# JerryX1110/Robust-Video-Object-Segmentation

Measured on AMD Instinct MI355X. Metric: frames/sec, AOC-Net matching + calibration hot path (480p, 3 objects), higher is better.
Workload: dtype f32; 1 GPU; cfg2: 121x213 stride-4 maps (480p), O=4 (3 objects + background), K=16 proxies, C=100, 60-frame clips, MEM_EVERY=5 (pool R=1..12), 20 Lloyd iterations, local windows 2..12, 10 IA gates + 4 conditioning blocks; sequences_per_gpu=2, proxy_mode=reference

## Files before the change

robust-video-object-segmentation_amd/csrc/dense_split.hip:

```cpp
#include <atomic>
#include <type_traits>

#include "aoc_common.h"

namespace {

typedef _Float16 f16x8 __attribute__((ext_vector_type(8)));
typedef float f32x16 __attribute__((ext_vector_type(16)));

constexpr int SP_KS = 7;
constexpr int SP_K = SP_KS * 16;
constexpr int SP_HALF = SP_KS * 2;
constexpr int SP_REC = 2 * SP_HALF;
constexpr int SP_NORM_SLOT = 100;
constexpr int SP_REST_SLOT = 104;
constexpr float SP_SCALE = 1024.0f;
constexpr float SP_QCONST = 32768.0f;
constexpr float SP_UNSCALE = -1.0f / 524288.0f;
constexpr int SP_TILE = 32;
constexpr int SP_NB = 4;
constexpr int SP_NQ = 2;

static_assert(SP_NORM_SLOT + 4 <= SP_K && SP_NORM_SLOT / 16 == SP_KS - 1 && (SP_NORM_SLOT % 16) + 4 <= 8, "norm slots live in the low half of the last k-step");
static_assert(SP_REST_SLOT / 16 == SP_KS - 1 && SP_REST_SLOT % 16 == 8, "the rest-norm slots are the first two halves of the last k-step's high chunk");

template <bool TILED>
__global__ __launch_bounds__(256) void split_rows_kernel(const float *__restrict__ x, int64_t n, int C, uint4 *__restrict__ rec,
                                                          float *__restrict__ sqnorm, int32_t *__restrict__ overflow) {
    const int64_t idx = (int64_t)blockIdx.x * blockDim.x + threadIdx.x;
    int64_t row;
    int ks;
    if (TILED) {
        const int64_t tile = idx / (SP_KS * 32);
        const int rem = (int)(idx - tile * (SP_KS * 32));
        ks = rem >> 5;
        row = tile * 32 + (rem & 31);
        if (tile * 32 >= n) return;
    } else {
        row = idx / SP_KS;
        ks = (int)(idx - row * SP_KS);
        if (row >= n) return;
    }
    const bool live = row < n;
    const float *xr = x + (size_t)(live ? row : n - 1) * C;
    _Float16 hi[16], lo[16];
    bool bad = false;
    {
        const int c4k = C >> 2;
        float4 kv[4];
#pragma unroll
        for (int q = 0; q < 4; ++q) kv[q] = reinterpret_cast<const float4 *>(xr)[min(ks * 4 + q, c4k - 1)];
#pragma unroll
        for (int q = 0; q < 4; ++q) {
            const bool in = ks * 4 + q < c4k;
            const float e4[4] = {kv[q].x, kv[q].y, kv[q].z, kv[q].w};
#pragma unroll
            for (int u = 0; u < 4; ++u) {
                const float v = in ? e4[u] * SP_SCALE : 0.0f;
                bad |= !(fabsf(v) <= 65000.0f);
                hi[q * 4 + u] = (_Float16)v;
                lo[q * 4 + u] = (_Float16)(v - (float)hi[q * 4 + u]);
            }
        }
    }
    if (ks == SP_KS - 1) {
        float s = 0.0f, sl = 0.0f, hr3 = 0.0f, hr4 = 0.0f;
        float4 rv[SP_NORM_SLOT / 4];
        const int c4n = C >> 2;
#pragma unroll
        for (int t4 = 0; t4 < SP_NORM_SLOT / 4; ++t4) rv[t4] = reinterpret_cast<const float4 *>(xr)[t4 < c4n ? t4 : c4n - 1];
#pragma unroll
        for (int t4 = 0; t4 < SP_NORM_SLOT / 4; ++t4) {
            if (t4 < c4n) {
// ... 89 lines not shown
        if (obj < 0 && t < base + nt) { obj = o; local = (int)(nt - 1 - (t - base)); }
        base += nt;
    }
    if (e == 0) *n_tiles = (int32_t)base;
    int32_t id = -1;
    if (obj >= 0) {
        const int pos = local * SP_TILE + i;
        id = obj_rows[obj_offsets[obj] + (pos < counts[obj] ? pos : local * SP_TILE)];
    }
    tile_rows[e] = id;
    if (i == 0) tile_obj[t] = obj;
}

__device__ __forceinline__ float max16(const f32x16 &a) {
    float m0 = __builtin_fmaxf(__builtin_fmaxf(a[0], a[1]), a[2]);
    float m1 = __builtin_fmaxf(__builtin_fmaxf(a[3], a[4]), a[5]);
    float m2 = __builtin_fmaxf(__builtin_fmaxf(a[6], a[7]), a[8]);
    float m3 = __builtin_fmaxf(__builtin_fmaxf(a[9], a[10]), a[11]);
    float m4 = __builtin_fmaxf(__builtin_fmaxf(a[12], a[13]), a[14]);
    m0 = __builtin_fmaxf(__builtin_fmaxf(m0, m1), m2);
    m3 = __builtin_fmaxf(__builtin_fmaxf(m3, m4), a[15]);
    return __builtin_fmaxf(m0, m3);
}

__device__ __forceinline__ uint32_t ord_enc(float f) {
    const uint32_t u = __float_as_uint(f);
    return (u & 0x80000000u) ? ~u : (u | 0x80000000u);
}
__device__ __forceinline__ float ord_dec(uint32_t u) {
    if (u == 0u) return -INFINITY;
    return __uint_as_float((u & 0x80000000u) ? (u & 0x7fffffffu) : ~u);
}
__device__ __forceinline__ uint32_t load_relaxed(const uint32_t *p) {
    return __hip_atomic_load(p, __ATOMIC_RELAXED, __HIP_MEMORY_SCOPE_AGENT);
}

#ifdef AOC_DEV
__device__ unsigned long long aoc_dev_block_times[4096 * 6];
#endif
__device__ unsigned long long g_prune_stats[8];

__device__ __forceinline__ void glds16(const void *gsrc, uint32_t lds_dst) {
    unsigned keep;
    asm volatile("s_mov_b32 %0, m0\n\ts_mov_b32 m0, %2\n\ts_nop 0\n\tglobal_load_lds_dwordx4 %1, off\n\ts_mov_b32 m0, %0"
                 : "=&s"(keep) : "v"(gsrc), "s"(lds_dst) : "memory");
}
__device__ __forceinline__ void glds4(const void *gsrc, uint32_t lds_dst) {
    unsigned keep;
    asm volatile("s_mov_b32 %0, m0\n\ts_mov_b32 m0, %2\n\ts_nop 0\n\tglobal_load_lds_dword %1, off\n\ts_mov_b32 m0, %0"
                 : "=&s"(keep) : "v"(gsrc), "s"(lds_dst) : "memory");
}

constexpr int SP_NBUF = 2;
__host__ __device__ constexpr int sp_chunk_bytes(int nb) { return nb * SP_TILE * SP_REC * 16; }
__host__ __device__ constexpr int sp_ids_off(int nb) { return SP_NBUF * sp_chunk_bytes(nb); }
__host__ __device__ constexpr int sp_obj_off(int nb) { return sp_ids_off(nb) + 2 * 512; }
__host__ __device__ constexpr int sp_bnd_off(int nb) { return sp_obj_off(nb) + 4 * 256; }
__host__ __device__ constexpr int sp_lds_bytes(int nw, int nb) { return sp_bnd_off(nb) + nw * SP_NQ * 256; }
constexpr int SP_TILE_SLACK = 2;

template <int NW, int CKPT, int NB = SP_NB>
__global__ __launch_bounds__(NW * 64, NB == 2 ? 2 : 1) void dense_prune_kernel(const uint4 *__restrict__ qrec, const float *__restrict__ q2, int64_t m,
                                                                     const uint4 *__restrict__ prec, const int32_t *__restrict__ tile_rows,
                                                                     const int32_t *__restrict__ tile_obj, const int32_t *__restrict__ n_tiles_ptr,
                                                                     const int32_t *__restrict__ gate, const uint32_t *__restrict__ pmax_bits,
                                                                     int n_obj, uint32_t *__restrict__ gbest, int dbg_arg, int q_tiled) {
    if (*gate) return;
#ifdef AOC_DEV
    const int dbg = dbg_arg;
#else
    constexpr int dbg = 0;
    (void)dbg_arg;
#endif
    extern __shared__ __attribute__((aligned(16))) uint4 lds4[];
    static_assert(SP_NQ == 2 && ((NB == 4 && (NW == 8 || NW == 4)) || (NB == 2 && NW == 4)),
                  "the step structure below is written for 4 tiles x 2 query tiles x 8 (or 4) waves, or 2 tiles x 2 query tiles x 4 waves (two workgroups per CU)");
    constexpr int SP_CHUNK_BYTES = sp_chunk_bytes(NB), SP_IDS_OFF = sp_ids_off(NB), SP_OBJ_OFF = sp_obj_off(NB), SP_BND_OFF = sp_bnd_off(NB);
    static_assert(CKPT == 0 || CKPT == 3 || CKPT == 4, "checkpoint after 3 or 4 k-steps (rest norms in slots 104 / 105), or none");
    constexpr int SP_DMA_PER_WAVE = SP_CHUNK_BYTES / 1024 / NW;
    constexpr int W_ID0 = NW / 2, W_ID1 = NW - 1, W_OBJ = 1;
    const uint32_t lds_base = (uint32_t)reinterpret_cast<uintptr_t>(lds4);
    const char *lds_bytes = reinterpret_cast<const char *>(lds4);

    int bx, by;
    {
        const int nb = gridDim.x * gridDim.y, lin = blockIdx.y * gridDim.x + blockIdx.x;
        const int xcd = lin & 7, slot = lin >> 3, q = nb >> 3, r = nb & 7;
        const int v = (xcd < r ? xcd * (q + 1) : r * (q + 1) + (xcd - r) * q) + slot;
        by = v / gridDim.x;
        bx = v - by * gridDim.x;
    }
    const int n_tiles = *n_tiles_ptr;
    const int ns = gridDim.y;
    if (by >= n_tiles) return;
    const int n_mine = (n_tiles - by + ns - 1) / ns;
    const int n_chunks = (n_mine + NB - 1) / NB;

    const int lane = aoc_lane(), wave = __builtin_amdgcn_readfirstlane(threadIdx.x >> 6);
    const int col = lane & 31, h = lane >> 5;
    const int64_t wave_row0 = (int64_t)bx * (NW * SP_NQ * 32) + (int64_t)wave * (SP_NQ * 32);

    const float pmax = sqrtf(__uint_as_float(*pmax_bits)) * 1.001f;
    const float plmax = __uint_as_float(*(pmax_bits - 2));
    f16x8 bh[SP_NQ][SP_KS], bl[SP_NQ][SP_KS];
    float eps[SP_NQ];
    bool valid[SP_NQ];
#pragma unroll
    for (int iq = 0; iq < SP_NQ; ++iq) {
        const int64_t row = wave_row0 + iq * 32 + col;
        valid[iq] = row < m;
        const int64_t rr = valid[iq] ? row : 0;
        const uint4 *r = q_tiled ? qrec + (size_t)(rr >> 5) * (2 * SP_KS * 64) + h * 32 + (rr & 31) : qrec + (size_t)rr * SP_REC + h;
        const int ks_step = q_tiled ? 64 : 2, plane_step = q_tiled ? SP_KS * 64 : SP_HALF;
#pragma unroll
        for (int ks = 0; ks < SP_KS; ++ks) {
            uint4 u = r[ks * ks_step], v = r[plane_step + ks * ks_step];
            if (!valid[iq]) { u = make_uint4(0, 0, 0, 0); v = make_uint4(0, 0, 0, 0); }
            bh[iq][ks] = __builtin_bit_cast(f16x8, u);
            bl[iq][ks] = __builtin_bit_cast(f16x8, v);
        }
        const float ql_own = (float)bh[iq][SP_KS - 1][SP_NORM_SLOT % 16 + 3];
        if (h == 0) {
            bh[iq][SP_KS - 1][SP_NORM_SLOT % 16 + 3] = (_Float16)0.0f;
            bh[iq][SP_KS - 1][SP_NORM_SLOT % 16] = (_Float16)SP_QCONST;
            bh[iq][SP_KS - 1][SP_NORM_SLOT % 16 + 1] = (_Float16)SP_QCONST;
            bh[iq][SP_KS - 1][SP_NORM_SLOT % 16 + 2] = (_Float16)SP_QCONST;
        } else {
            if (CKPT != 3) bh[iq][SP_KS - 1][0] = (_Float16)0.0f;
            if (CKPT != 4) bh[iq][SP_KS - 1][1] = (_Float16)0.0f;
        }
        const float qn = valid[iq] ? sqrtf(q2[row]) : 0.0f;
        const float ql = valid[iq] ? __shfl(ql_own, col) : 0.0f;
        eps[iq] = (1026.0f * (qn * plmax + ql * pmax) + 8.0f * pmax * pmax + (CKPT != 0 ? 16.0f * qn * pmax : 0.0f) + 8.0f) * ((dbg & 64) ? 0.4f : 1.0f);
    }

    uint32_t dma_plan[SP_DMA_PER_WAVE];
#pragma unroll
    for (int k = 0; k < SP_DMA_PER_WAVE; ++k) {
        const int j = (wave * SP_DMA_PER_WAVE + k) * 64 + lane;
        const int r = j / SP_REC, pos = j - r * SP_REC;
        dma_plan[k] = ((uint32_t)r << 16) | (uint32_t)((pos ^ ((r >> 3) & 3)) * 16);
    }
    const char *prec_bytes = reinterpret_cast<const char *>(prec);
    auto dma_meta = [&](int chunk) {
        const int i0 = chunk * NB;
        if (wave == W_ID0 || (NB == 4 && wave == W_ID1)) {
            const int i = i0 + (wave == W_ID1 ? 2 : 0) + (lane >> 5);
            const int t = min(by + i * ns, n_tiles);
            glds4(tile_rows + (size_t)t * SP_TILE + (lane & 31), lds_base + SP_IDS_OFF + (chunk & 1) * 512 + (wave == W_ID1 ? 256 : 0));
        }
        if (wave == W_OBJ) glds4(tile_obj + min(by + (i0 + (lane & (NB - 1))) * ns, n_tiles), lds_base + SP_OBJ_OFF + (chunk & 3) * 256);
    };
    auto dma_rows = [&](int chunk) {
        const int32_t *ids = reinterpret_cast<const int32_t *>(lds_bytes + SP_IDS_OFF + (chunk & 1) * 512);
        const uint32_t dst = lds_base + (uint32_t)(chunk % SP_NBUF) * SP_CHUNK_BYTES + (uint32_t)(wave * SP_DMA_PER_WAVE) * 1024u;
        int id[SP_DMA_PER_WAVE];
#pragma unroll
        for (int k = 0; k < SP_DMA_PER_WAVE; ++k) id[k] = ids[dma_plan[k] >> 16];
#pragma unroll
        for (int k = 0; k < SP_DMA_PER_WAVE; ++k)
            glds16(prec_bytes + (size_t)(uint32_t)max(id[k], 0) * (SP_REC * 16) + (dma_plan[k] & 0xffffu), dst + (uint32_t)k * 1024u);
    };

    float best[SP_NQ], shared[SP_NQ];
    uint32_t grow[SP_NQ];
#pragma unroll
    for (int iq = 0; iq < SP_NQ; ++iq) {
        grow[iq] = valid[iq] ? (uint32_t)(wave_row0 + iq * 32 + col) * (uint32_t)n_obj : 0u;
        best[iq] = INFINITY;
        shared[iq] = INFINITY;
    }
    int cur = -1;
    unsigned n_rescored = 0, n_any = 0, n_seen = 0, n_dead = 0;
    unsigned long long cyc[6] = {0, 0, 0, 0, 0, 0};
    unsigned long long t_prev = 0;
    auto stamp = [&]() -> unsigned long long { return (dbg & 4096) ? __builtin_amdgcn_s_memtime() : 0ull; };
    auto dma_bound = [&]() {
#pragma unroll
        for (int iq = 0; iq < SP_NQ; ++iq) {
            unsigned keep;
            asm volatile("s_mov_b32 %0, m0\n\ts_mov_b32 m0, %2\n\ts_nop 0\n\tglobal_load_lds_dword %1, off sc1\n\ts_mov_b32 m0, %0"
                         : "=&s"(keep) : "v"(gbest + grow[iq] + max(cur, 0)), "s"(lds_base + SP_BND_OFF + (uint32_t)(wave * SP_NQ + iq) * 256u) : "memory");
        }
    };
    auto switch_object = [&](int o) {
        cur = o;
        uint32_t u[SP_NQ];
#pragma unroll
        for (int iq = 0; iq < SP_NQ; ++iq) u[iq] = load_relaxed(gbest + grow[iq] + cur);
#pragma unroll
        for (int iq = 0; iq < SP_NQ; ++iq) {
            best[iq] = valid[iq] ? -INFINITY : INFINITY;
            shared[iq] = valid[iq] ? ord_dec(u[iq]) : INFINITY;
        }
    };

#ifdef AOC_DEV
    const int blk_lin = blockIdx.y * gridDim.x + blockIdx.x;
    const bool blk_rec = (dbg & 32768) && threadIdx.x == 0 && blk_lin < 4096;
    if (blk_rec) aoc_dev_block_times[blk_lin * 6 + 0] = wall_clock64();
#endif
    dma_meta(0);
    dma_meta(1);
    __builtin_amdgcn_s_waitcnt(0x0f70);
    __builtin_amdgcn_s_barrier();
    dma_rows(0);
    __builtin_amdgcn_s_waitcnt(0x0f70);
    __builtin_amdgcn_s_barrier();

    const int xs = (col >> 3) & 3;
    const uint32_t row_off = (uint32_t)col * (SP_REC * 16);
    const uint32_t sw0 = row_off + (uint32_t)((h ^ xs) * 16), sw2 = row_off + (uint32_t)(((2 + h) ^ xs) * 16);
    auto frag = [&](const char *tile_base, int e) -> f16x8 {
        const uint32_t off = ((e & 2) ? sw2 : sw0) + (uint32_t)((e & ~3) * 16);
        return __builtin_bit_cast(f16x8, *reinterpret_cast<const uint4 *>(tile_base + off));
    };
    auto ks_of = [&](int kk) { return (kk + SP_KS - 1) % SP_KS; };
#ifdef AOC_DEV
    if (blk_rec) aoc_dev_block_times[blk_lin * 6 + 1] = wall_clock64();
#endif

    for (int s = 0; s < n_chunks; ++s) {
        const unsigned long long t_s0 = stamp();
        const int4 objs = *reinterpret_cast<const int4 *>(lds_bytes + SP_OBJ_OFF + (s & 3) * 256);
        const int bound_obj = (dbg & 32) ? -3 : cur;
        if (!(dbg & 32)) dma_bound();
        dma_meta(s + 2);
        if (!(dbg & 4)) dma_rows(s + 1);

        const char *chunk_base = lds_bytes + (s % SP_NBUF) * SP_CHUNK_BYTES;
        const int n_here = min(NB, n_mine - s * NB);
        f16x8 pre0 = frag(chunk_base, 2 * ks_of(0)), pre1 = frag(chunk_base, 2 * ks_of(1));
        const uint32_t objs_packed = (uint32_t)__builtin_amdgcn_readfirstlane((objs.x & 0xff) | ((objs.y & 0xff) << 8) | ((objs.z & 0xff) << 16) | ((objs.w & 0xff) << 24));
        t_prev = stamp();
        cyc[4] += t_prev - t_s0;
#pragma unroll 1
        for (int t = 0; t < n_here; ++t) {
            const char *tile_base = chunk_base + t * (SP_TILE * SP_REC * 16);
            const int o = (int)((objs_packed >> (8 * t)) & 0xffu);
            if (o != cur) switch_object(o);
            const unsigned long long t_0 = stamp();
            cyc[3] += t_0 - t_prev;
            f32x16 acc[SP_NQ];
#pragma unroll
            for (int iq = 0; iq < SP_NQ; ++iq)
#pragma unroll
                for (int r = 0; r < 16; ++r) acc[iq][r] = 0.0f;
            bool live[SP_NQ] = {true, true};
            if constexpr (CKPT == 0) {
                f16x8 af[3];
                af[0] = pre0;
                af[1] = pre1;
#pragma unroll
                for (int kk = 0; kk < SP_KS; ++kk) {
                    if (kk + 2 < SP_KS && !(dbg & 512)) af[(kk + 2) % 3] = frag(tile_base, 2 * ks_of(kk + 2));
#pragma unroll
                    for (int iq = 0; iq < SP_NQ; ++iq)
                        acc[iq] = __builtin_amdgcn_mfma_f32_32x32x16_f16(af[kk % 3], bh[iq][ks_of(kk)], acc[iq], 0, 0, 0);
                }
                if (t + 1 < n_here) {
                    pre0 = frag(tile_base + SP_TILE * SP_REC * 16, 2 * ks_of(0));
                    pre1 = frag(tile_base + SP_TILE * SP_REC * 16, 2 * ks_of(1));
                }
            } else {
                f16x8 af[3];
                af[0] = pre0;
                af[1] = frag(tile_base, 2 * ks_of(1));
                const uint32_t a6d0 = __builtin_bit_cast(uint4, pre0).x;
#pragma unroll
                for (int kk = 0; kk < CKPT; ++kk) {
                    if (kk + 2 < CKPT) af[(kk + 2) % 3] = frag(tile_base, 2 * ks_of(kk + 2));
#pragma unroll
                    for (int iq = 0; iq < SP_NQ; ++iq)
                        acc[iq] = __builtin_amdgcn_mfma_f32_32x32x16_f16(af[kk % 3], bh[iq][ks_of(kk)], acc[iq], 0, 0, 0);
                }
                if (t + 1 < n_here) pre0 = frag(tile_base + SP_TILE * SP_REC * 16, 2 * ks_of(0));
#pragma unroll
                for (int iq = 0; iq < SP_NQ; ++iq) {
                    const float cm = max16(acc[iq]);
                    live[iq] = (__builtin_amdgcn_ballot_w64(cm + eps[iq] >= __builtin_fmaxf(best[iq], shared[iq])) != 0ull) || (dbg & 128);
                    if (!live[iq]) n_dead += 1;
                }
                if (live[0] || live[1]) {
                    uint4 c4 = make_uint4(0u, 0u, 0u, 0u);
                    if (h == 1) c4.x = (CKPT == 3) ? ((a6d0 & 0x0000ffffu) ^ 0x00008000u) : ((a6d0 & 0xffff0000u) ^ 0x80000000u);
                    const f16x8 a6c = __builtin_bit_cast(f16x8, c4);
                    auto phase2 = [&](auto q0, auto q1) {
                        constexpr bool Q0 = decltype(q0)::value, Q1 = decltype(q1)::value;
                        f16x8 ar[3];
                        ar[0] = frag(tile_base, 2 * ks_of(CKPT));
                        ar[1] = frag(tile_base, 2 * ks_of(CKPT + 1));
                        if (Q0) acc[0] = __builtin_amdgcn_mfma_f32_32x32x16_f16(a6c, bh[0][SP_KS - 1], acc[0], 0, 0, 0);
                        if (Q1) acc[1] = __builtin_amdgcn_mfma_f32_32x32x16_f16(a6c, bh[1][SP_KS - 1], acc[1], 0, 0, 0);
#pragma unroll
                        for (int kk = CKPT; kk < SP_KS; ++kk) {
                            if (kk + 2 < SP_KS) ar[(kk + 2 - CKPT) % 3] = frag(tile_base, 2 * ks_of(kk + 2));
                            if (Q0) acc[0] = __builtin_amdgcn_mfma_f32_32x32x16_f16(ar[(kk - CKPT) % 3], bh[0][ks_of(kk)], acc[0], 0, 0, 0);
                            if (Q1) acc[1] = __builtin_amdgcn_mfma_f32_32x32x16_f16(ar[(kk - CKPT) % 3], bh[1][ks_of(kk)], acc[1], 0, 0, 0);
                        }
                    };
                    if (live[0] && live[1]) phase2(std::true_type{}, std::true_type{});
                    else if (live[0]) phase2(std::true_type{}, std::false_type{});
                    else phase2(std::false_type{}, std::true_type{});
                }
            }
            const unsigned long long t_1 = stamp();
            cyc[0] += t_1 - t_0;
            bool want[SP_NQ];
#pragma unroll
            for (int iq = 0; iq < SP_NQ; ++iq) {
                want[iq] = false;
                if (live[iq] && !(dbg & 256)) {
                    const float cm = max16(acc[iq]);
                    want[iq] = __builtin_amdgcn_ballot_w64(cm + eps[iq] >= __builtin_fmaxf(best[iq], shared[iq])) != 0ull;
                }
            }
            n_seen += 1;
            const unsigned long long t_2 = stamp();
            cyc[1] += t_2 - t_1;
            t_prev = t_2;
            if ((want[0] || want[1]) && !(dbg & 2)) {
                n_any += 1;
#pragma unroll
                for (int iq = 0; iq < SP_NQ; ++iq) {
                    if (want[iq]) {
                        n_rescored += 1;
                        if (dbg & 65536) {
                            if (cur == 0) cyc[0] += 1;
                            else if (cur == 1) cyc[1] += 1;
                            else if (cur == 2) cyc[2] += 1;
                        }
                        f16x8 ah[3], al[3];
#pragma unroll
                        for (int kk = 0; kk < 2; ++kk) {
                            ah[kk] = frag(tile_base, 2 * ks_of(kk));
                            al[kk] = frag(tile_base, 2 * SP_KS + 2 * ks_of(kk));
                        }
#pragma unroll
                        for (int kk = 0; kk < SP_KS; ++kk) {
                            if (kk + 2 < SP_KS) {
                                ah[(kk + 2) % 3] = frag(tile_base, 2 * ks_of(kk + 2));
                                al[(kk + 2) % 3] = frag(tile_base, 2 * SP_KS + 2 * ks_of(kk + 2));
                            }
                            acc[iq] = __builtin_amdgcn_mfma_f32_32x32x16_f16(ah[kk % 3], bl[iq][ks_of(kk)], acc[iq], 0, 0, 0);
                            acc[iq] = __builtin_amdgcn_mfma_f32_32x32x16_f16(al[kk % 3], bh[iq][ks_of(kk)], acc[iq], 0, 0, 0);
                        }
                        const float ex = max16(acc[iq]);
                        if (ex > best[iq]) {
                            best[iq] = ex;
                            if (ex > shared[iq] && !(dbg & 1)) atomicMax(gbest + grow[iq] + cur, ord_enc(ex));
                        }
                    }
                }
                t_prev = stamp();
                cyc[2] += t_prev - t_2;
            }
        }
        const unsigned long long t_s1 = stamp();

        __builtin_amdgcn_s_waitcnt(0x0f70);
        uint32_t seen[SP_NQ];
#pragma unroll
        for (int iq = 0; iq < SP_NQ; ++iq)
            seen[iq] = *reinterpret_cast<const volatile uint32_t *>(lds_bytes + SP_BND_OFF + (wave * SP_NQ + iq) * 256 + lane * 4);
        __builtin_amdgcn_s_waitcnt(0xc07f);
        if (!(dbg & 8)) __builtin_amdgcn_s_barrier();
        if (bound_obj == cur && cur >= 0) {
#pragma unroll
            for (int iq = 0; iq < SP_NQ; ++iq)
                if (valid[iq]) shared[iq] = __builtin_fmaxf(shared[iq], ord_dec(seen[iq]));
        }
        cyc[5] += stamp() - t_s1;
#ifdef AOC_DEV
        if (blk_rec && s == 0) aoc_dev_block_times[blk_lin * 6 + 2] = wall_clock64();
#endif
    }
#ifdef AOC_DEV
    if (blk_rec) {
        aoc_dev_block_times[blk_lin * 6 + 3] = wall_clock64();
        aoc_dev_block_times[blk_lin * 6 + 4] = n_seen;
        aoc_dev_block_times[blk_lin * 6 + 5] = n_rescored;
    }
#endif
    if (lane == 0) {
        atomicAdd(&g_prune_stats[0], (unsigned long long)n_seen * SP_NQ);
        atomicAdd(&g_prune_stats[1], (unsigned long long)n_rescored);
        atomicAdd(&g_prune_stats[2], (unsigned long long)n_any);
        atomicAdd(&g_prune_stats[3], (unsigned long long)n_seen);
        atomicAdd(&g_prune_stats[4], (unsigned long long)n_dead);
        if (dbg & (4096 | 65536)) {
            const int b = (dbg & 8192) ? 3 : 0;
            atomicAdd(&g_prune_stats[5], cyc[b]);
            atomicAdd(&g_prune_stats[6], cyc[b + 1]);
            atomicAdd(&g_prune_stats[7], cyc[b + 2]);
        }
    }
}

#ifndef AOC_DENSE_Q4
#define AOC_DENSE_Q4 0
#endif
#if defined(AOC_DEV) || AOC_DENSE_Q4
constexpr int Q4_NW = 4, Q4_NQ = 4;
#ifndef AOC_Q4_DBG
#define AOC_Q4_DBG 0
#endif
// ... 290 lines not shown

__global__ __launch_bounds__(256) void dense_split_finalize_kernel(uint32_t *__restrict__ gbest, int64_t m, int n_obj,
                                                                    const int32_t *__restrict__ counts, const int32_t *__restrict__ gate,
                                                                    const float *__restrict__ q2, const float *__restrict__ obj_bias,
                                                                    float *__restrict__ out, int64_t pstride, int64_t ostride, int transform) {
    if (*gate) return;
    const int64_t row = (int64_t)blockIdx.x * blockDim.x + threadIdx.x;
    if (row >= m) return;
    const float qq = q2[row];
    float own[16];
    int n_kept = 0;
#pragma unroll
    for (int o = 0; o < 16; ++o) {
        own[o] = INFINITY;
        if (o < n_obj && counts[o] > 0) {
            own[o] = qq + SP_UNSCALE * ord_dec(gbest[(size_t)row * n_obj + o]);
            gbest[(size_t)row * n_obj + o] = 0u;
            n_kept += counts[o];
        }
    }
#pragma unroll
    for (int o = 0; o < 16; ++o) {
        if (o < n_obj) {
            float others = INFINITY;
#pragma unroll
            for (int o2 = 0; o2 < 16; ++o2)
                if (o2 != o && o2 < n_obj) others = fminf(others, own[o2]);
            float v = fminf(own[o], others + AOC_PAD_DISTANCE);
            if (n_kept == 0) v = transform ? 1.0f : INFINITY;
            else if (transform) v = aoc_proto_transform(v, obj_bias ? obj_bias[o] : 0.0f);
            out[row * pstride + o * ostride] = v;
        }
    }
}

__global__ void split_gate_refresh_kernel(const int32_t *__restrict__ overflow, int32_t *__restrict__ gate) {
    if (*overflow) atomicOr(gate, 1);
}

inline int split_waves() {
    static const int nw = AOC_DEV_ENV_INT("AOC_DENSE_WAVES", 8) == 4 ? 4 : 8;
    return nw;
}
#if defined(AOC_DEV) || AOC_DENSE_Q4
inline bool split_q4() {
    static const bool q4 = AOC_DEV_ENV_INT("AOC_DENSE_Q4", AOC_DENSE_Q4) != 0 && split_waves() == 8;
    return q4;
}
#endif
inline int split_tiles_per_chunk() {
    static const int nb = (AOC_DEV_ENV_INT("AOC_DENSE_NB", SP_NB) == 2 && split_waves() == 4) ? 2 : SP_NB;
    return nb;
}
inline int split_nsplit(int64_t m) {
    const int64_t rpb = (int64_t)split_waves() * SP_NQ * 32;
    const int64_t row_blocks = (m + rpb - 1) / rpb;
    const int wg_per_cu = split_tiles_per_chunk() == 2 ? 2 : 1;
    static const int max_rounds = AOC_DEV_ENV_INT("AOC_DENSE_ROUNDS", 2);
    const int n_cu = (aoc_stream_cus() > 0 ? aoc_stream_cus() : 256) * wg_per_cu;
    int best = 1;
    double best_eff = 0.0;
    for (int k = 1; k <= max_rounds; ++k) {
        int64_t ns = ((int64_t)n_cu * k) / row_blocks;
        if (ns < 1) ns = 1;
        if (ns > 64) ns = 64;
        const int64_t blocks = row_blocks * ns;
        const int64_t rounds = (blocks + n_cu - 1) / n_cu;
        const double eff = (double)blocks / ((double)n_cu * rounds);
        if (eff >= best_eff - 0.005) { best_eff = eff > best_eff ? eff : best_eff; best = (int)ns; }
    }
    return best;
}

inline int split_ckpt() {
    static const int c = AOC_DEV_ENV_INT("AOC_DENSE_CKPT", 0);
    return (c == 3 || c == 4) ? c : 0;
}

struct SplitWs {
    int32_t *gate, *n_tiles, *tile_rows, *tile_obj;
    uint32_t *pmax, *gbest;
    void *fp32_ws;
    size_t fp32_bytes, total;
    int64_t tile_capacity;
};
inline SplitWs split_carve(void *base, int64_t m, int64_t n, int n_obj) {
    SplitWs w;
    char *p = static_cast<char *>(base);
    size_t off = 0;
    auto take = [&](size_t bytes) { char *r = p ? p + off : nullptr; off += aoc_align_up(bytes, 256); return r; };
    w.tile_capacity = (n + SP_TILE - 1) / SP_TILE + n_obj + SP_TILE_SLACK;
    w.gate = reinterpret_cast<int32_t *>(take(16));
    w.n_tiles = w.gate ? w.gate + 2 : nullptr;
    w.pmax = w.gate ? reinterpret_cast<uint32_t *>(w.gate + 3) : nullptr;
    w.tile_rows = reinterpret_cast<int32_t *>(take((size_t)w.tile_capacity * SP_TILE * sizeof(int32_t)));
    w.tile_obj = reinterpret_cast<int32_t *>(take((size_t)w.tile_capacity * sizeof(int32_t)));
    w.gbest = reinterpret_cast<uint32_t *>(take((size_t)m * n_obj * sizeof(uint32_t)));
    w.fp32_bytes = aoc_dense_match_workspace_bytes(m, n, n_obj);
    w.fp32_ws = take(w.fp32_bytes);
    w.total = off;
    return w;
}

}

extern "C" {
// ... 23 lines not shown
    const int64_t total = (n + 31) / 32 * 32 * SP_KS;
    hipLaunchKernelGGL(split_rows_kernel<true>, dim3((unsigned)((total + 255) / 256)), dim3(256), 0, aoc_hip_stream(stream), x, n, C,
                       static_cast<uint4 *>(records), sqnorm, overflow_flag);
    AOC_RETURN_IF_LAUNCH_FAILED();
    return AOC_OK;
}

size_t aoc_dense_match_split_workspace_bytes(int64_t m, int64_t n, int n_obj) {
    if (m < 1 || n < 1 || n_obj < 1) return 0;
    return split_carve(nullptr, m, n, n_obj).total;
}

int aoc_dense_match_min_split(const float *query, const void *query_rec, const float *query_sqnorm, int query_rec_tiled, int64_t m, int C, const float *pool,
                              const void *pool_rec, const int32_t *overflow_flag, int64_t n, const uint32_t *right_bits,
                              const uint32_t *wrong_bits, const int32_t *fg_rows, const int32_t *obj_rows, const int32_t *counts,
                              const int32_t *obj_offsets, const float *obj_bias, int n_obj, float *out, int64_t out_pixel_stride,
                              int64_t out_obj_stride, int transform, void *workspace, size_t workspace_bytes, aoc_stream_t stream) {
    return aoc_dense_match_min_split_cached(query, query_rec, query_sqnorm, query_rec_tiled, m, C, pool, pool_rec, overflow_flag, n, right_bits, wrong_bits,
                                            fg_rows, obj_rows, counts, obj_offsets, obj_bias, n_obj, out, out_pixel_stride, out_obj_stride, transform, workspace,
                                            workspace_bytes, 0, stream);
}

int aoc_dense_match_min_split_cached(const float *query, const void *query_rec, const float *query_sqnorm, int query_rec_tiled, int64_t m, int C, const float *pool,
                                     const void *pool_rec, const int32_t *overflow_flag, int64_t n, const uint32_t *right_bits,
                                     const uint32_t *wrong_bits, const int32_t *fg_rows, const int32_t *obj_rows, const int32_t *counts,
                                     const int32_t *obj_offsets, const float *obj_bias, int n_obj, float *out, int64_t out_pixel_stride,
                                     int64_t out_obj_stride, int transform, void *workspace, size_t workspace_bytes, int reuse_plan, aoc_stream_t stream) {
    if (!query || !query_rec || !query_sqnorm || !pool || !pool_rec || !overflow_flag || !right_bits || !wrong_bits || !fg_rows ||
        !obj_rows || !counts || !obj_offsets || !out || !workspace)
        return AOC_ERR_INVALID_ARG;
    if (m < 1 || n < 1 || n >= (1ll << 31) - 4096 || n_obj < 1) return AOC_ERR_INVALID_ARG;
    if (aoc_split_record_bytes(C) == 0 || n_obj > 16) return AOC_ERR_UNSUPPORTED;
    if (workspace_bytes < aoc_dense_match_split_workspace_bytes(m, n, n_obj)) return AOC_ERR_WORKSPACE;
    hipStream_t st = aoc_hip_stream(stream);
    const SplitWs w = split_carve(workspace, m, n, n_obj);
    if (reuse_plan) {
        hipLaunchKernelGGL(split_gate_refresh_kernel, dim3(1), dim3(1), 0, st, overflow_flag, w.gate);
    } else {
        if (hipMemsetAsync(w.gate, 0, 16, st) != hipSuccess) return AOC_ERR_LAUNCH;
        if (hipMemsetAsync(w.gbest, 0, (size_t)m * n_obj * sizeof(uint32_t), st) != hipSuccess) return AOC_ERR_LAUNCH;
        const int64_t plan_threads = w.tile_capacity * SP_TILE > n ? w.tile_capacity * SP_TILE : n;
        hipLaunchKernelGGL(split_plan_kernel, dim3((unsigned)((plan_threads + 255) / 256)), dim3(256), 0, st, obj_rows, counts, obj_offsets, n_obj, n,
                           right_bits, wrong_bits, overflow_flag, static_cast<const uint4 *>(pool_rec), w.tile_capacity, w.tile_rows, w.tile_obj,
                           w.n_tiles, w.gate, w.pmax);
    }
    static const bool seeds = AOC_DEV_ENV_INT("AOC_DENSE_SEED", AOC_DENSE_SEED) != 0;
    if (seeds && n >= m)
        hipLaunchKernelGGL(dense_seed_kernel, dim3((unsigned)((m * 8 + 255) / 256)), dim3(256), 0, st, query, query_sqnorm, m, C, pool, n, right_bits, n_obj, w.gate,
                           w.gbest);
    const int ns = split_nsplit(m);
    const int nw = split_waves();
    const int64_t rpb = (int64_t)nw * SP_NQ * 32;
    const dim3 grid((unsigned)((m + rpb - 1) / rpb), ns);
    const int nb = split_tiles_per_chunk();
    const size_t lds = sp_lds_bytes(nw, nb);
#if defined(AOC_DEV) || AOC_DENSE_Q4
    if (split_q4()) {
        static const bool q4_ok = hipFuncSetAttribute(reinterpret_cast<const void *>(dense_prune_q4_kernel), hipFuncAttributeMaxDynamicSharedMemorySize,
                                                      q4_lds_bytes()) == hipSuccess;
        if (!q4_ok) return AOC_ERR_LAUNCH;
        const AocDenseProbe probe4 = aoc_take_dense_probe();
        if (probe4.start) (void)hipEventRecord(probe4.start, st);
        hipLaunchKernelGGL(dense_prune_q4_kernel, grid, dim3(Q4_NW * 64), q4_lds_bytes(), st, static_cast<const uint4 *>(query_rec), query_sqnorm, m,
                           static_cast<const uint4 *>(pool_rec), w.tile_rows, w.tile_obj, w.n_tiles, w.gate, w.pmax, n_obj, w.gbest, query_rec_tiled ? 1 : 0);
        if (probe4.stop) (void)hipEventRecord(probe4.stop, st);
        hipLaunchKernelGGL(dense_split_finalize_kernel, dim3((unsigned)((m + 255) / 256)), dim3(256), 0, st, w.gbest, m, n_obj, counts, w.gate,
                           query_sqnorm, obj_bias, out, out_pixel_stride, out_obj_stride, transform);
        AOC_RETURN_IF_LAUNCH_FAILED();
        return aoc_dense_match_min_gated(query, m, C, pool, fg_rows, counts + n_obj, n, wrong_bits, obj_bias, n_obj, out, out_pixel_stride,
                                         out_obj_stride, transform, w.fp32_ws, w.fp32_bytes, w.gate, stream);
    }
#endif
    const AocDenseProbe probe = aoc_take_dense_probe();
    static const int dbg = AOC_DEV_ENV_INT("AOC_DENSE_DEBUG", 0);
    const int ckpt = split_ckpt();
    int launched = 0;
#define AOC_DENSE_LAUNCH(NW_, CK_, NB_)                                                                                                                     \
    if (!launched && nw == NW_ && ckpt == CK_ && nb == NB_) {                                                                                               \
        static const bool lds_ok = hipFuncSetAttribute(reinterpret_cast<const void *>(dense_prune_kernel<NW_, CK_, NB_>),                                  \
                                                       hipFuncAttributeMaxDynamicSharedMemorySize, (int)lds) == hipSuccess;                                \
        if (!lds_ok) return AOC_ERR_LAUNCH;                                                                                                                 \
        if (probe.start) (void)hipEventRecord(probe.start, st);                                                                                             \
        hipLaunchKernelGGL((dense_prune_kernel<NW_, CK_, NB_>), grid, dim3(NW_ * 64), lds, st, static_cast<const uint4 *>(query_rec), query_sqnorm, m,           \
                           static_cast<const uint4 *>(pool_rec), w.tile_rows, w.tile_obj, w.n_tiles, w.gate, w.pmax, n_obj, w.gbest, dbg,                   \
                           query_rec_tiled ? 1 : 0);                                                                                                        \
        launched = 1;                                                                                                                                       \
    }
    AOC_DENSE_LAUNCH(8, 0, 4)
#ifdef AOC_DEV
    AOC_DENSE_LAUNCH(8, 3, 4)
    AOC_DENSE_LAUNCH(8, 4, 4)
    AOC_DENSE_LAUNCH(4, 0, 4)
    AOC_DENSE_LAUNCH(4, 3, 4)
    AOC_DENSE_LAUNCH(4, 0, 2)
#endif
#undef AOC_DENSE_LAUNCH
    if (!launched) return AOC_ERR_UNSUPPORTED;
    if (probe.stop) (void)hipEventRecord(probe.stop, st);
    hipLaunchKernelGGL(dense_split_finalize_kernel, dim3((unsigned)((m + 255) / 256)), dim3(256), 0, st, w.gbest, m, n_obj, counts, w.gate,
                       query_sqnorm, obj_bias, out, out_pixel_stride, out_obj_stride, transform);
    AOC_RETURN_IF_LAUNCH_FAILED();
    return aoc_dense_match_min_gated(query, m, C, pool, fg_rows, counts + n_obj, n, wrong_bits, obj_bias, n_obj, out, out_pixel_stride,
                                     out_obj_stride, transform, w.fp32_ws, w.fp32_bytes, w.gate, stream);
}

static std::atomic<int> g_stream_cus{0};
int aoc_set_stream_cus(int n_cus) {
    if (n_cus < 0) return AOC_ERR_INVALID_ARG;
    g_stream_cus.store(n_cus, std::memory_order_relaxed);
    return AOC_OK;
}

int aoc_dense_prune_stats(uint64_t *out4, int reset) {
    if (!out4) return AOC_ERR_INVALID_ARG;
    uint64_t v[8];
    const int rc = aoc_dense_prune_stats_ex(v, reset);
    for (int i = 0; i < 4 && rc == AOC_OK; ++i) out4[i] = v[i];
    return rc;
}

#ifdef AOC_DEV
int aoc_dev_dense_block_times(uint64_t *out, int n_words) {
    if (!out || n_words < 1 || n_words > 4096 * 6) return AOC_ERR_INVALID_ARG;
    return hipMemcpyFromSymbol(out, HIP_SYMBOL(aoc_dev_block_times), (size_t)n_words * sizeof(uint64_t)) == hipSuccess ? AOC_OK : AOC_ERR_LAUNCH;
}
#endif

int aoc_dense_prune_stats_ex(uint64_t *out8, int reset) {
    if (!out8) return AOC_ERR_INVALID_ARG;
    unsigned long long v[8] = {0, 0, 0, 0, 0, 0, 0, 0};
    if (hipMemcpyFromSymbol(v, HIP_SYMBOL(g_prune_stats), sizeof(v)) != hipSuccess) return AOC_ERR_LAUNCH;
    for (int i = 0; i < 8; ++i) out8[i] = v[i];
    if (reset) {
        const unsigned long long z[8] = {0, 0, 0, 0, 0, 0, 0, 0};
        if (hipMemcpyToSymbol(HIP_SYMBOL(g_prune_stats), z, sizeof(z)) != hipSuccess) return AOC_ERR_LAUNCH;
    }
    return AOC_OK;
}

}

static thread_local int t_stream_cus = 0;
int aoc_stream_cus() { return t_stream_cus > 0 ? t_stream_cus : g_stream_cus.load(std::memory_order_relaxed); }
int aoc_stream_cus_scope(int n_cus) {
    const int before = t_stream_cus;
    t_stream_cus = n_cus > 0 ? n_cus : 0;
    return before;
// ... 2 lines not shown
```

Before: 427.3 frames/s.

## Stage only hi-half pool records in LDS ring, fetch lo half on rescore

The dense prune kernel now streams only the high-precision half of each pool record into the LDS ring, so the same ring holds 8 tiles per chunk instead of 4. The low half, needed only when a tile must be rescored, is loaded straight from global memory at that point. This halves LDS staging traffic and doubles the tiles handled per chunk. In exchange, rescores now wait on global loads, and the tile-id and object metadata layouts change to fit 8 tiles.

New measurement: 443.7 frames/s (median of 6 runs). 3.8% higher.

```diff
diff --git a/robust-video-object-segmentation_amd/csrc/dense_split.hip b/robust-video-object-segmentation_amd/csrc/dense_split.hip
--- a/robust-video-object-segmentation_amd/csrc/dense_split.hip
+++ b/robust-video-object-segmentation_amd/csrc/dense_split.hip
@@ -19,6 +19,7 @@
 constexpr float SP_UNSCALE = -1.0f / 524288.0f;
 constexpr int SP_TILE = 32;
 constexpr int SP_NB = 4;
+constexpr int SP_NB_HI = 8;
 constexpr int SP_NQ = 2;
 
 static_assert(SP_NORM_SLOT + 4 <= SP_K && SP_NORM_SLOT / 16 == SP_KS - 1 && (SP_NORM_SLOT % 16) + 4 <= 8, "norm slots live in the low half of the last k-step");
@@ -214,14 +215,16 @@
 }
 
 constexpr int SP_NBUF = 2;
-__host__ __device__ constexpr int sp_chunk_bytes(int nb) { return nb * SP_TILE * SP_REC * 16; }
-__host__ __device__ constexpr int sp_ids_off(int nb) { return SP_NBUF * sp_chunk_bytes(nb); }
-__host__ __device__ constexpr int sp_obj_off(int nb) { return sp_ids_off(nb) + 2 * 512; }
-__host__ __device__ constexpr int sp_bnd_off(int nb) { return sp_obj_off(nb) + 4 * 256; }
-__host__ __device__ constexpr int sp_lds_bytes(int nw, int nb) { return sp_bnd_off(nb) + nw * SP_NQ * 256; }
+__host__ __device__ constexpr int sp_row_chunks(bool hi) { return hi ? SP_HALF : SP_REC; }
+__host__ __device__ constexpr int sp_chunk_bytes(int nb, bool hi = false) { return nb * SP_TILE * sp_row_chunks(hi) * 16; }
+__host__ __device__ constexpr int sp_ids_off(int nb, bool hi = false) { return SP_NBUF * sp_chunk_bytes(nb, hi); }
+__host__ __device__ constexpr int sp_obj_off(int nb, bool hi = false) { return sp_ids_off(nb, hi) + (hi ? 3 * 1024 : 2 * 512); }
+__host__ __device__ constexpr int sp_bnd_off(int nb, bool hi = false) { return sp_obj_off(nb, hi) + 4 * 256; }
+__host__ __device__ constexpr int sp_lds_bytes(int nw, int nb, bool hi = false) { return sp_bnd_off(nb, hi) + nw * SP_NQ * 256; }
+static_assert(sp_chunk_bytes(SP_NB_HI, true) == sp_chunk_bytes(SP_NB) && sp_lds_bytes(8, SP_NB_HI, true) == 122880, "the hi-plane ring has the size of the record ring; 120 KiB per workgroup");
 constexpr int SP_TILE_SLACK = 2;
 
-template <int NW, int CKPT, int NB = SP_NB>
+template <int NW, int CKPT, int NB = SP_NB, bool HI = false>
 __global__ __launch_bounds__(NW * 64, NB == 2 ? 2 : 1) void dense_prune_kernel(const uint4 *__restrict__ qrec, const float *__restrict__ q2, int64_t m,
                                                                      const uint4 *__restrict__ prec, const int32_t *__restrict__ tile_rows,
                                                                      const int32_t *__restrict__ tile_obj, const int32_t *__restrict__ n_tiles_ptr,
@@ -235,9 +238,13 @@
     (void)dbg_arg;
 #endif
     extern __shared__ __attribute__((aligned(16))) uint4 lds4[];
-    static_assert(SP_NQ == 2 && ((NB == 4 && (NW == 8 || NW == 4)) || (NB == 2 && NW == 4)),
-                  "the step structure below is written for 4 tiles x 2 query tiles x 8 (or 4) waves, or 2 tiles x 2 query tiles x 4 waves (two workgroups per CU)");
-    constexpr int SP_CHUNK_BYTES = sp_chunk_bytes(NB), SP_IDS_OFF = sp_ids_off(NB), SP_OBJ_OFF = sp_obj_off(NB), SP_BND_OFF = sp_bnd_off(NB);
+    static_assert(SP_NQ == 2 && (HI ? (NB == 8 && NW == 8 && CKPT == 0) : ((NB == 4 && (NW == 8 || NW == 4)) || (NB == 2 && NW == 4))),
+                  "the step structure below is written for 8 hi-plane tiles x 2 query tiles x 8 waves, for 4 record tiles x 2 query tiles x 8 (or 4) waves, or for "
+                  "2 record tiles x 2 query tiles x 4 waves (two workgroups per CU)");
+    constexpr int SP_CHUNK_BYTES = sp_chunk_bytes(NB, HI), SP_IDS_OFF = sp_ids_off(NB, HI), SP_OBJ_OFF = sp_obj_off(NB, HI), SP_BND_OFF = sp_bnd_off(NB, HI);
+    constexpr int ROW_CHUNKS = sp_row_chunks(HI), ROW_BYTES = ROW_CHUNKS * 16, TILE_BYTES = SP_TILE * ROW_BYTES;
+    constexpr int IDS_SLOTS = HI ? 3 : 2, IDS_SLOT_BYTES = HI ? 1024 : 512;
+    constexpr int SWZ_MASK = HI ? 1 : 3;
     static_assert(CKPT == 0 || CKPT == 3 || CKPT == 4, "checkpoint after 3 or 4 k-steps (rest norms in slots 104 / 105), or none");
     constexpr int SP_DMA_PER_WAVE = SP_CHUNK_BYTES / 1024 / NW;
     constexpr int W_ID0 = NW / 2, W_ID1 = NW - 1, W_OBJ = 1;
@@ -300,13 +307,18 @@
 #pragma unroll
     for (int k = 0; k < SP_DMA_PER_WAVE; ++k) {
         const int j = (wave * SP_DMA_PER_WAVE + k) * 64 + lane;
-        const int r = j / SP_REC, pos = j - r * SP_REC;
-        dma_plan[k] = ((uint32_t)r << 16) | (uint32_t)((pos ^ ((r >> 3) & 3)) * 16);
+        const int r = j / ROW_CHUNKS, pos = j - r * ROW_CHUNKS;
+        dma_plan[k] = ((uint32_t)r << 16) | (uint32_t)((pos ^ ((r >> 3) & SWZ_MASK)) * 16);
     }
     const char *prec_bytes = reinterpret_cast<const char *>(prec);
     auto dma_meta = [&](int chunk) {
         const int i0 = chunk * NB;
-        if (wave == W_ID0 || (NB == 4 && wave == W_ID1)) {
+        if constexpr (HI) {
+            if (wave == W_ID0) {
+                const int t = min(by + (i0 + (lane >> 3)) * ns, n_tiles);
+                glds16(tile_rows + (size_t)t * SP_TILE + (lane & 7) * 4, lds_base + SP_IDS_OFF + (chunk % IDS_SLOTS) * IDS_SLOT_BYTES);
+            }
+        } else if (wave == W_ID0 || (NB == 4 && wave == W_ID1)) {
             const int i = i0 + (wave == W_ID1 ? 2 : 0) + (lane >> 5);
             const int t = min(by + i * ns, n_tiles);
             glds4(tile_rows + (size_t)t * SP_TILE + (lane & 31), lds_base + SP_IDS_OFF + (chunk & 1) * 512 + (wave == W_ID1 ? 256 : 0));
@@ -314,7 +326,7 @@
         if (wave == W_OBJ) glds4(tile_obj + min(by + (i0 + (lane & (NB - 1))) * ns, n_tiles), lds_base + SP_OBJ_OFF + (chunk & 3) * 256);
     };
     auto dma_rows = [&](int chunk) {
-        const int32_t *ids = reinterpret_cast<const int32_t *>(lds_bytes + SP_IDS_OFF + (chunk & 1) * 512);
+        const int32_t *ids = reinterpret_cast<const int32_t *>(lds_bytes + SP_IDS_OFF + (chunk % IDS_SLOTS) * IDS_SLOT_BYTES);
         const uint32_t dst = lds_base + (uint32_t)(chunk % SP_NBUF) * SP_CHUNK_BYTES + (uint32_t)(wave * SP_DMA_PER_WAVE) * 1024u;
         int id[SP_DMA_PER_WAVE];
 #pragma unroll
@@ -370,9 +382,9 @@
     __builtin_amdgcn_s_waitcnt(0x0f70);
     __builtin_amdgcn_s_barrier();
 
-    const int xs = (col >> 3) & 3;
-    const uint32_t row_off = (uint32_t)col * (SP_REC * 16);
-    const uint32_t sw0 = row_off + (uint32_t)((h ^ xs) * 16), sw2 = row_off + (uint32_t)(((2 + h) ^ xs) * 16);
+    const int xs = (col >> 3) & SWZ_MASK;
+    const uint32_t row_off = (uint32_t)col * ROW_BYTES;
+    const uint32_t sw0 = row_off + (uint32_t)((h ^ xs) * 16), sw2 = HI ? sw0 + 32u : row_off + (uint32_t)(((2 + h) ^ xs) * 16);
     auto frag = [&](const char *tile_base, int e) -> f16x8 {
         const uint32_t off = ((e & 2) ? sw2 : sw0) + (uint32_t)((e & ~3) * 16);
         return __builtin_bit_cast(f16x8, *reinterpret_cast<const uint4 *>(tile_base + off));
@@ -385,6 +397,8 @@
     for (int s = 0; s < n_chunks; ++s) {
         const unsigned long long t_s0 = stamp();
         const int4 objs = *reinterpret_cast<const int4 *>(lds_bytes + SP_OBJ_OFF + (s & 3) * 256);
+        int4 objs_b = make_int4(0, 0, 0, 0);
+        if constexpr (NB == 8) objs_b = *reinterpret_cast<const int4 *>(lds_bytes + SP_OBJ_OFF + (s & 3) * 256 + 16);
         const int bound_obj = (dbg & 32) ? -3 : cur;
         if (!(dbg & 32)) dma_bound();
         dma_meta(s + 2);
@@ -393,12 +407,15 @@
         const char *chunk_base = lds_bytes + (s % SP_NBUF) * SP_CHUNK_BYTES;
         const int n_here = min(NB, n_mine - s * NB);
         f16x8 pre0 = frag(chunk_base, 2 * ks_of(0)), pre1 = frag(chunk_base, 2 * ks_of(1));
-        const uint32_t objs_packed = (uint32_t)__builtin_amdgcn_readfirstlane((objs.x & 0xff) | ((objs.y & 0xff) << 8) | ((objs.z & 0xff) << 16) | ((objs.w & 0xff) << 24));
+        const uint32_t objs_lo = (uint32_t)__builtin_amdgcn_readfirstlane((objs.x & 0xff) | ((objs.y & 0xff) << 8) | ((objs.z & 0xff) << 16) | ((objs.w & 0xff) << 24));
+        const uint32_t objs_hi = (uint32_t)__builtin_amdgcn_readfirstlane((objs_b.x & 0xff) | ((objs_b.y & 0xff) << 8) | ((objs_b.z & 0xff) << 16) | ((objs_b.w & 0xff) << 24));
+        const uint64_t objs_packed = NB == 8 ? ((uint64_t)objs_hi << 32) | objs_lo : (uint64_t)objs_lo;
+        const int32_t *ids_now = reinterpret_cast<const int32_t *>(lds_bytes + SP_IDS_OFF + (s % IDS_SLOTS) * IDS_SLOT_BYTES);
         t_prev = stamp();
         cyc[4] += t_prev - t_s0;
 #pragma unroll 1
         for (int t = 0; t < n_here; ++t) {
-            const char *tile_base = chunk_base + t * (SP_TILE * SP_REC * 16);
+            const char *tile_base = chunk_base + t * TILE_BYTES;
             const int o = (int)((objs_packed >> (8 * t)) & 0xffu);
             if (o != cur) switch_object(o);
             const unsigned long long t_0 = stamp();
@@ -421,8 +438,8 @@
                         acc[iq] = __builtin_amdgcn_mfma_f32_32x32x16_f16(af[kk % 3], bh[iq][ks_of(kk)], acc[iq], 0, 0, 0);
                 }
                 if (t + 1 < n_here) {
-                    pre0 = frag(tile_base + SP_TILE * SP_REC * 16, 2 * ks_of(0));
-                    pre1 = frag(tile_base + SP_TILE * SP_REC * 16, 2 * ks_of(1));
+                    pre0 = frag(tile_base + TILE_BYTES, 2 * ks_of(0));
+                    pre1 = frag(tile_base + TILE_BYTES, 2 * ks_of(1));
                 }
             } else {
                 f16x8 af[3];
@@ -436,7 +453,7 @@
                     for (int iq = 0; iq < SP_NQ; ++iq)
                         acc[iq] = __builtin_amdgcn_mfma_f32_32x32x16_f16(af[kk % 3], bh[iq][ks_of(kk)], acc[iq], 0, 0, 0);
                 }
-                if (t + 1 < n_here) pre0 = frag(tile_base + SP_TILE * SP_REC * 16, 2 * ks_of(0));
+                if (t + 1 < n_here) pre0 = frag(tile_base + TILE_BYTES, 2 * ks_of(0));
 #pragma unroll
                 for (int iq = 0; iq < SP_NQ; ++iq) {
                     const float cm = max16(acc[iq]);
@@ -483,37 +500,49 @@
             t_prev = t_2;
             if ((want[0] || want[1]) && !(dbg & 2)) {
                 n_any += 1;
-#pragma unroll
-                for (int iq = 0; iq < SP_NQ; ++iq) {
-                    if (want[iq]) {
-                        n_rescored += 1;
-                        if (dbg & 65536) {
-                            if (cur == 0) cyc[0] += 1;
-                            else if (cur == 1) cyc[1] += 1;
-                            else if (cur == 2) cyc[2] += 1;
+                f16x8 alg[SP_KS];
+                auto load_lo = [&]() {
+                    if constexpr (HI) {
+                        const int id = ids_now[t * SP_TILE + col];
+                        const uint4 *lo = reinterpret_cast<const uint4 *>(prec_bytes + (size_t)(uint32_t)max(id, 0) * (SP_REC * 16) + SP_HALF * 16) + h;
+#pragma unroll
+                        for (int kk = 0; kk < SP_KS; ++kk) alg[kk] = __builtin_bit_cast(f16x8, lo[2 * ks_of(kk)]);
+                        __builtin_amdgcn_s_waitcnt(0x0f70);
+                    }
+                };
+                auto rescore = [&](auto iq_c) {
+                    constexpr int iq = decltype(iq_c)::value;
+                    n_rescored += 1;
+                    if (dbg & 65536) {
+                        if (cur == 0) cyc[0] += 1;
+                        else if (cur == 1) cyc[1] += 1;
+                        else if (cur == 2) cyc[2] += 1;
+                    }
+                    f16x8 ah[3], al[3];
+#pragma unroll
+                    for (int kk = 0; kk < 2; ++kk) {
+                        ah[kk] = frag(tile_base, 2 * ks_of(kk));
+                        if constexpr (!HI) al[kk] = frag(tile_base, 2 * SP_KS + 2 * ks_of(kk));
+                    }
+#pragma unroll
+                    for (int kk = 0; kk < SP_KS; ++kk) {
+                        if (kk + 2 < SP_KS) {
+                            ah[(kk + 2) % 3] = frag(tile_base, 2 * ks_of(kk + 2));
+                            if constexpr (!HI) al[(kk + 2) % 3] = frag(tile_base, 2 * SP_KS + 2 * ks_of(kk + 2));
                         }
-                        f16x8 ah[3], al[3];
-#pragma unroll
-                        for (int kk = 0; kk < 2; ++kk) {
-                            ah[kk] = frag(tile_base, 2 * ks_of(kk));
-                            al[kk] = frag(tile_base, 2 * SP_KS + 2 * ks_of(kk));
-                        }
-#pragma unroll
-                        for (int kk = 0; kk < SP_KS; ++kk) {
-                            if (kk + 2 < SP_KS) {
-                                ah[(kk + 2) % 3] = frag(tile_base, 2 * ks_of(kk + 2));
-                                al[(kk + 2) % 3] = frag(tile_base, 2 * SP_KS + 2 * ks_of(kk + 2));
-                            }
-                            acc[iq] = __builtin_amdgcn_mfma_f32_32x32x16_f16(ah[kk % 3], bl[iq][ks_of(kk)], acc[iq], 0, 0, 0);
-                            acc[iq] = __builtin_amdgcn_mfma_f32_32x32x16_f16(al[kk % 3], bh[iq][ks_of(kk)], acc[iq], 0, 0, 0);
-                        }
-                        const float ex = max16(acc[iq]);
-                        if (ex > best[iq]) {
-                            best[iq] = ex;
-                            if (ex > shared[iq] && !(dbg & 1)) atomicMax(gbest + grow[iq] + cur, ord_enc(ex));
-                        }
+                        acc[iq] = __builtin_amdgcn_mfma_f32_32x32x16_f16(ah[kk % 3], bl[iq][ks_of(kk)], acc[iq], 0, 0, 0);
+                        if constexpr (HI) acc[iq] = __builtin_amdgcn_mfma_f32_32x32x16_f16(alg[kk], bh[iq][ks_of(kk)], acc[iq], 0, 0, 0);
+                        else acc[iq] = __builtin_amdgcn_mfma_f32_32x32x16_f16(al[kk % 3], bh[iq][ks_of(kk)], acc[iq], 0, 0, 0);
                     }
-                }
+                    const float ex = max16(acc[iq]);
+                    if (ex > best[iq]) {
+                        best[iq] = ex;
+                        if (ex > shared[iq] && !(dbg & 1)) atomicMax(gbest + grow[iq] + cur, ord_enc(ex));
+                    }
+                };
+                load_lo();
+                if (want[0]) rescore(std::integral_constant<int, 0>{});
+                if (want[1]) rescore(std::integral_constant<int, 1>{});
                 t_prev = stamp();
                 cyc[2] += t_prev - t_2;
             }
@@ -910,6 +939,11 @@
     static const int nb = (AOC_DEV_ENV_INT("AOC_DENSE_NB", SP_NB) == 2 && split_waves() == 4) ? 2 : SP_NB;
     return nb;
 }
+inline int split_ckpt();
+inline bool split_hi_ring() {
+    static const bool hi = AOC_DEV_ENV_INT("AOC_DENSE_HI", 1) != 0 && split_waves() == 8 && split_tiles_per_chunk() == SP_NB && split_ckpt() == 0;
+    return hi;
+}
 inline int split_nsplit(int64_t m) {
     const int64_t rpb = (int64_t)split_waves() * SP_NQ * 32;
     const int64_t row_blocks = (m + rpb - 1) / rpb;
@@ -1039,8 +1073,9 @@
     const int nw = split_waves();
     const int64_t rpb = (int64_t)nw * SP_NQ * 32;
     const dim3 grid((unsigned)((m + rpb - 1) / rpb), ns);
-    const int nb = split_tiles_per_chunk();
-    const size_t lds = sp_lds_bytes(nw, nb);
+    const bool hi = split_hi_ring();
+    const int nb = hi ? SP_NB_HI : split_tiles_per_chunk();
+    const size_t lds = sp_lds_bytes(nw, nb, hi);
 #if defined(AOC_DEV) || AOC_DENSE_Q4
     if (split_q4()) {
         static const bool q4_ok = hipFuncSetAttribute(reinterpret_cast<const void *>(dense_prune_q4_kernel), hipFuncAttributeMaxDynamicSharedMemorySize,
@@ -1062,24 +1097,25 @@
     static const int dbg = AOC_DEV_ENV_INT("AOC_DENSE_DEBUG", 0);
     const int ckpt = split_ckpt();
     int launched = 0;
-#define AOC_DENSE_LAUNCH(NW_, CK_, NB_)                                                                                                                     \
-    if (!launched && nw == NW_ && ckpt == CK_ && nb == NB_) {                                                                                               \
-        static const bool lds_ok = hipFuncSetAttribute(reinterpret_cast<const void *>(dense_prune_kernel<NW_, CK_, NB_>),                                  \
+#define AOC_DENSE_LAUNCH(NW_, CK_, NB_, HI_)                                                                                                                  \
+    if (!launched && nw == NW_ && ckpt == CK_ && nb == NB_ && hi == HI_) {                                                                                        \
+        static const bool lds_ok = hipFuncSetAttribute(reinterpret_cast<const void *>(dense_prune_kernel<NW_, CK_, NB_, HI_>),                             \
                                                        hipFuncAttributeMaxDynamicSharedMemorySize, (int)lds) == hipSuccess;                                \
         if (!lds_ok) return AOC_ERR_LAUNCH;                                                                                                                 \
         if (probe.start) (void)hipEventRecord(probe.start, st);                                                                                             \
-        hipLaunchKernelGGL((dense_prune_kernel<NW_, CK_, NB_>), grid, dim3(NW_ * 64), lds, st, static_cast<const uint4 *>(query_rec), query_sqnorm, m,           \
+        hipLaunchKernelGGL((dense_prune_kernel<NW_, CK_, NB_, HI_>), grid, dim3(NW_ * 64), lds, st, static_cast<const uint4 *>(query_rec), query_sqnorm, m,      \
                            static_cast<const uint4 *>(pool_rec), w.tile_rows, w.tile_obj, w.n_tiles, w.gate, w.pmax, n_obj, w.gbest, dbg,                   \
                            query_rec_tiled ? 1 : 0);                                                                                                        \
         launched = 1;                                                                                                                                       \
     }
-    AOC_DENSE_LAUNCH(8, 0, 4)
+    AOC_DENSE_LAUNCH(8, 0, 8, true)
 #ifdef AOC_DEV
-    AOC_DENSE_LAUNCH(8, 3, 4)
-    AOC_DENSE_LAUNCH(8, 4, 4)
-    AOC_DENSE_LAUNCH(4, 0, 4)
-    AOC_DENSE_LAUNCH(4, 3, 4)
-    AOC_DENSE_LAUNCH(4, 0, 2)
+    AOC_DENSE_LAUNCH(8, 0, 4, false)
+    AOC_DENSE_LAUNCH(8, 3, 4, false)
+    AOC_DENSE_LAUNCH(8, 4, 4, false)
+    AOC_DENSE_LAUNCH(4, 0, 4, false)
+    AOC_DENSE_LAUNCH(4, 3, 4, false)
+    AOC_DENSE_LAUNCH(4, 0, 2, false)
 #endif
 #undef AOC_DENSE_LAUNCH
     if (!launched) return AOC_ERR_UNSUPPORTED;
```
